# Roywangj/AdaptPoint

Hardware: AMD Instinct MI355X
Metric: set-abstraction fwd+bwd point-clouds/sec (B=32,N=1024) (higher is better)
Workload: dtype bf16

## Files before the change

adaptpoint_amd/_lib.py:

```python
import ctypes
import os

_HERE = os.path.dirname(os.path.abspath(__file__))
LIB_PATH = os.path.join(_HERE, "libadaptpoint_amd.so")
if os.environ.get("APN_LIB_PATH"):
    if os.environ.get("APN_ALLOW_UNSAFE_LIB") != "1":
        raise RuntimeError("APN_LIB_PATH is for diagnostic builds: set APN_ALLOW_UNSAFE_LIB=1 with it")
    LIB_PATH = os.path.abspath(os.environ["APN_LIB_PATH"])
REQUIRED_BUILD_FLAGS = ("-ffp-contract=off", "-fno-slp-vectorize")

_c_int, _c_float, _c_void_p = ctypes.c_int, ctypes.c_float, ctypes.c_void_p
_c_double = ctypes.c_double
_c_longlong = ctypes.c_longlong

SIGNATURES = {
    "apn_version": [],
    "apn_furthest_point_sampling": [_c_int] * 3 + [_c_void_p] * 4,
    "apn_ball_query": [_c_int] * 3 + [_c_float, _c_int] + [_c_void_p] * 4,
    "apn_group_points": [_c_int] * 5 + [_c_void_p] * 4,
    "apn_group_points_grad": [_c_int] * 5 + [_c_void_p] * 4,
    "apn_gather_points": [_c_int] * 4 + [_c_void_p] * 4,
    "apn_gather_points_grad": [_c_int] * 4 + [_c_void_p] * 4,
    "apn_resample_points": [_c_int] * 6 + [_c_void_p] * 6,
    "apn_three_nn": [_c_int] * 3 + [_c_void_p] * 5,
# ... 30 lines not shown
                       + [_c_void_p] * 3 + [_c_int] + [_c_void_p] * 8,
    "apn_sa_bwd_main": [_c_int] * 4 + [_c_float] + [_c_void_p] * 11 + [_c_double, _c_int] + [_c_void_p] * 9,
    "apn_sa_bwd_weight_rows": [_c_int] * 2,
    "apn_sa_bwd_point_grads": [_c_int] * 3 + [_c_void_p] * 7 + [_c_double, _c_int] + [_c_void_p] * 2 + [_c_int]
                              + [_c_void_p] * 4 + [_c_float] + [_c_void_p] * 5,
    "apn_sa_bwd_finalize": [_c_void_p, _c_int, _c_float, _c_void_p, _c_void_p, _c_int, _c_void_p, _c_void_p, _c_int]
                           + [_c_void_p] * 11,
    "apn_sa_forward_seq": ([_c_int] * 5 + [_c_float] + [_c_void_p] * 12
                           + [_c_void_p] * 5 + [_c_float, _c_float, _c_int]
                           + [_c_void_p] * 5 + [_c_float, _c_float, _c_int]
                           + [_c_double, _c_int] + [_c_void_p] * 11 + [_c_longlong, _c_void_p]),
    "apn_sa_backward_seq": ([_c_int] * 5 + [_c_float] + [_c_void_p] * 15 + [_c_int] * 3
                            + [_c_double] + [_c_void_p] + [_c_longlong] * 3 + [_c_void_p]
                            + [_c_longlong]
                            + [_c_void_p] * 26),
    "apn_attention_small_max": [],
    "apn_attention_small_fwd": [_c_int] * 3 + [_c_void_p] * 5,
    "apn_attention_small_bwd": [_c_int] * 3 + [_c_void_p] * 8,
    "apn_attention_prep": [_c_int] * 3 + [_c_void_p] * 4 + [_c_int, _c_void_p],
    "apn_attention_fwd": [_c_int] * 3 + [_c_void_p] * 4,
    "apn_attention_bwd": [_c_int] * 3 + [_c_void_p] * 9,
    "apn_pointset_group_rows": [_c_int] * 3,
    "apn_pointset_group_max": [_c_int] * 5 + [_c_void_p] * 8,
    "apn_pointset_group_max_grad": [_c_int] * 5 + [_c_void_p] * 9,
    "apn_sa_wide_grid": [_c_int] * 2,
    "apn_sa_wide_colsum_chunks": [_c_int] * 2,
    "apn_sa_wide_colsum": [_c_void_p, _c_int, _c_int, _c_void_p, _c_void_p, _c_void_p],
    "apn_sa_wide_tilemap_ints": [_c_int] * 2,
    "apn_sa_wide_tilemap": [_c_int] * 3 + [_c_void_p] * 3,
    "apn_sa_wide_tilemap_many": [_c_int] * 4 + [_c_void_p] * 3,
    "apn_sa_rowmap_many": [_c_int] * 4 + [_c_void_p] * 6,
    "apn_sa_rowmap_ints": [_c_int] * 2,
    "apn_sa_rowmap_places": [_c_int] * 3,
    "apn_sa_wide_stats1": [_c_int] * 4 + [_c_void_p] * 6,
    "apn_sa_wide_fwd_main": [_c_int] * 5 + [_c_void_p] * 11,
    "apn_sa_wide_bwd_main": [_c_int] * 5 + [_c_void_p] * 15,
    "apn_sa_wide_wgrad_fused": [_c_int],
    "apn_sa_wide_image": [_c_void_p, _c_int, _c_int, _c_void_p, _c_int, _c_int, _c_int, _c_void_p, _c_void_p],
    "apn_sa_wide_bwd_prep_rows": [_c_int] * 2,
    "apn_sa_wide_bwd_prep": [_c_int] * 3 + [_c_void_p] + [_c_longlong] * 3 + [_c_void_p] * 7,
    "apn_sa_wide_consts2": [_c_void_p, _c_int, _c_void_p, _c_int, _c_void_p, _c_double, _c_int] + [_c_void_p] * 4,
    "apn_sa_wide_consts1": [_c_void_p, _c_int, _c_void_p, _c_int, _c_void_p, _c_double, _c_int] + [_c_void_p] * 4,
    "apn_sa_wide_point_terms": [_c_int] * 4 + [_c_void_p] * 5 + [_c_int, _c_float] + [_c_void_p] * 7,
    "apn_sa_wide_wgrad_splits": [_c_int] * 3,
    "apn_sa_wide_csr": [_c_int] * 3 + [_c_void_p] * 9,
    "apn_sa_wide_fwd_prep": [_c_int] * 6 + [_c_float] + [_c_void_p] * 13,
    "apn_sa_wide_fwd_prep_rows": [_c_int] * 3,
    "apn_sa_wide_out": [_c_int] * 3 + [_c_void_p] * 2 + [_c_int] + [_c_void_p] * 3 + [_c_int] + [_c_void_p] * 2,
    "apn_sa_wide_bwd_mid": [_c_void_p, _c_int, _c_void_p, _c_int, _c_int, _c_void_p, _c_double, _c_int] + [_c_void_p] * 7,
    "apn_sa_wide_bwd_fin": [_c_void_p, _c_int, _c_void_p, _c_int, _c_int, _c_void_p, _c_double, _c_int] + [_c_void_p] * 8,
    "apn_sa_wide_point_grads_rows": [_c_int] * 2,
    "apn_sa_wide_point_grads_cols": [_c_int] * 3,
    "apn_sa_wide_point_grads": [_c_int] * 5 + [_c_float] + [_c_void_p] * 13 + [_c_int] + [_c_void_p] * 9,
    "apn_sa_wide_colsum_f32": [_c_void_p, _c_int, _c_int, _c_void_p, _c_void_p],
    "apn_sa_wide_wgrad": [_c_int] * 5 + [_c_void_p] * 7 + [_c_int] + [_c_void_p] * 2,
    "apn_pw_conv_tiles": [_c_int] * 2,
    "apn_pw_conv_forward": [_c_int] * 5 + [_c_void_p] * 5,
    "apn_pw_bn_act": [_c_int] * 3 + [_c_void_p] * 2 + [_c_int] + [_c_void_p] * 2 + [_c_float] * 2 + [_c_int] * 2
                     + [_c_void_p] * 6,
    "apn_pw_bn_act_grad_splits": [_c_int] * 2,
    "apn_pw_bn_act_grad": [_c_int] * 3 + [_c_void_p] * 3 + [_c_int] * 2 + [_c_void_p] * 5,
    "apn_pw_conv_grad_input": [_c_int] * 5 + [_c_void_p] * 4,
    "apn_pw_conv_grad_weight_splits": [_c_int] * 4,
    "apn_pw_conv_grad_weight": [_c_int] * 5 + [_c_void_p] * 5,
    "apn_deform_forward": [_c_int] * 3 + [_c_void_p] * 6 + [_c_float] + [_c_void_p] * 4,
    "apn_deform_backward": [_c_int] * 3 + [_c_void_p] * 4 + [_c_float] + [_c_void_p] * 7,
# ... 82 lines not shown
_lib = None


class ExtensionMissing(RuntimeError):
    pass


def load():
    global _lib
    if _lib is not None:
        return _lib
    if not os.path.exists(LIB_PATH):
        raise ExtensionMissing(
            f"{LIB_PATH} not found: build it with `python -m adaptpoint_amd.build` "
            "(hipcc --offload-arch=gfx950). There is no fallback path.")
    lib = ctypes.CDLL(LIB_PATH)
    for name, argtypes in SIGNATURES.items():
        fn = getattr(lib, name)
        fn.argtypes = argtypes
        fn.restype = _c_int
    lib.apn_error_string.argtypes = [_c_int]
    lib.apn_error_string.restype = ctypes.c_char_p
    lib.apn_build_flags.argtypes = []
    lib.apn_build_flags.restype = ctypes.c_char_p
    flags = lib.apn_build_flags().decode("utf-8", "replace").split()
    missing = [f for f in REQUIRED_BUILD_FLAGS if f not in flags]
    if missing and os.environ.get("APN_ALLOW_UNSAFE_LIB") != "1":
        raise ExtensionMissing(f"{LIB_PATH} was built without {missing} (its flags: {' '.join(flags)}): rebuild with "
                               "`python -m adaptpoint_amd.build --force`")
    _lib = lib
    return lib


def check(code, what):
    if code != 0:
        msg = load().apn_error_string(code).decode("utf-8", "replace")
        raise RuntimeError(f"{what} failed: {msg} (code {code})")
```

adaptpoint_amd/build.py:

```python
import argparse
import os
import shutil
import subprocess
import sys

HERE = os.path.dirname(os.path.abspath(__file__))
CSRC = os.path.join(HERE, "csrc")
OBJ = os.path.join(HERE, "csrc", "build")
LIB = os.path.join(HERE, "libadaptpoint_amd.so")
ARCH = "gfx950"
SOURCES = ["capi.hip", "fps.hip", "ball_query.hip", "group_points.hip", "interpolate.hip", "sa_fused.hip", "sa_glue.hip", "sa_seq.hip", "sa_geo.hip", "sa_wide.hip", "sa_wide_glue.hip", "sa_wide_dense.hip", "pointwise.hip", "feature_prop.hip", "spectral.hip", "augment.hip", "pointset_group.hip", "attention.hip", "online_aug.hip", "cloud_transform.hip", "cls_metrics.hip", "local_aggr.hip", "knn.hip", "edge_conv.hip", "chamfer.hip", "emd.hip", "pointops.hip", "point_transformer.hip", "voxel_grid.hip"]
HEADERS = ["apn_common.h", "apn_mfma.h", "sa_chain.h", "ball_query_body.h", "anchor_rotation.h", "lds_bitonic.h", "knn_list.h",
           os.path.join("..", "..", "include", "adaptpoint_amd.h")]
CXXFLAGS = ["-O3", "-std=c++17", "-fPIC", "-ffp-contract=off", "-fno-fast-math", "-fno-slp-vectorize",
            "-fvisibility=hidden", "-Wall", "-Wno-unused-command-line-argument"] + os.environ.get("APN_EXTRA_CXXFLAGS", "").split()
REQUIRED_FLAGS = ("-ffp-contract=off", "-fno-slp-vectorize")
FORBIDDEN_FLAGS = ("-fslp-vectorize", "-ffp-contract=fast", "-ffp-contract=on", "-ffast-math", "-Ofast")


NO_SLP = ["-fno-slp-vectorize"]
FILE_FLAGS = {}


def hipcc():
    exe = shutil.which("hipcc") or "/opt/rocm/bin/hipcc"
    if not os.path.exists(exe):
        raise RuntimeError("hipcc not found; libadaptpoint_amd.so cannot be built")
    return exe


def _newer(target, deps):
    if not os.path.exists(target):
        return False
    t = os.path.getmtime(target)
    return all(os.path.getmtime(d) <= t for d in deps)


def flag_line(src):
    return " ".join([*CXXFLAGS, *FILE_FLAGS.get(os.path.basename(src), [])])


def check_flags():
    bad = [f for f in CXXFLAGS if f in FORBIDDEN_FLAGS] + [f for f in REQUIRED_FLAGS if f not in CXXFLAGS]
    if bad:
# ... 56 lines not shown
```

adaptpoint_amd/csrc/capi.hip:

```cpp
#include "apn_common.h"

extern "C" int apn_version(void) { return 100;  }

#ifndef APN_BUILD_FLAGS
#define APN_BUILD_FLAGS "unknown"
#endif
extern "C" const char *apn_build_flags(void) { return APN_BUILD_FLAGS; }

extern "C" const char *apn_error_string(int code) {
    if (code == APN_OK) return "success";
    if (code == APN_EINVAL) return "invalid argument (negative size, null pointer or size beyond the launch limits)";
    return hipGetErrorString((hipError_t)code);
}

namespace apn {
__global__ void stamp_kernel(unsigned long long *stamps, int slot) { stamps[slot] = wall_clock64(); }
}

extern "C" int apn_debug_stamp(void *stamps, int slot, void *stream) {
    if (stamps == nullptr || slot < 0) return APN_EINVAL;
    hipLaunchKernelGGL(apn::stamp_kernel, dim3(1), dim3(1), 0, (hipStream_t)stream, (unsigned long long *)stamps, slot);
    return (int)hipGetLastError();
}

namespace apn {
__global__ __launch_bounds__(256) void vgpr_hold_kernel(int turns, unsigned long long *bad) {
    __shared__ unsigned long long slot[4];
    const unsigned lane = threadIdx.x;
    unsigned r[24];
#pragma unroll
    for (int i = 0; i < 24; ++i) r[i] = 0x10000u * (unsigned)(i + 1) + lane * 131u + blockIdx.x;
    if (lane < 4) slot[lane] = 0ull;
    __syncthreads();
    for (int t = 0; t < turns; ++t) {
#pragma unroll
        for (int i = 0; i < 24; ++i) asm volatile("" : "+v"(r[i]));
        if ((lane & 63) == (unsigned)(t & 63))
            atomicMax(&slot[t & 3], ((unsigned long long)r[0] << 32) | (unsigned)t);
        asm volatile("s_waitcnt lgkmcnt(0)\n\ts_barrier" ::: "memory");
        const unsigned k = (unsigned)slot[t & 3];
        if (k == 0xFFFFFFFFu) r[23] ^= 1u;
    }
#pragma unroll
    for (int i = 0; i < 24; ++i) {
// ... 91 lines not shown
```

adaptpoint_amd/fused.py:

```python
import torch
import torch.distributed as dist
import torch.nn as nn

from . import _lib
from . import ops as _ops

C_IN, C_MID, C_OUT, K_NS = 32, 32, 64, 32
DETERMINISTIC = True

PRECISION = "bf16x3"
_PREC = {"bf16": 1, "bf16x3": 2}

PER_KERNEL_LAUNCH = False


def covers(B, N, M, K, C, w1, w2, biased=False, momenta=()):
    return (C == C_IN and K == K_NS and tuple(w1) == (C_MID, C_IN + 3) and tuple(w2) == (C_OUT, C_MID) and not biased
            and (M is None or M <= N) and B <= 65535 and all(m is not None for m in momenta))


def supported(p, f, idx_or_k, conv1, conv2, bns=(), npoint=None):
    k = idx_or_k.shape[2] if torch.is_tensor(idx_or_k) else int(idx_or_k)
    m = idx_or_k.shape[1] if torch.is_tensor(idx_or_k) else npoint
    return (f.is_cuda and f.dtype == torch.float32 and p.dtype == torch.float32
            and covers(p.shape[0], p.shape[1], m, k, f.shape[1], conv1.weight.shape[:2], conv2.weight.shape[:2],
                       conv1.bias is not None or conv2.bias is not None, [bn.momentum for bn in bns]))


_FN = {}


def _call(name, dev, *args, stream=None):
    fn = _FN.get(name)
    if fn is None:
        fn = _FN[name] = getattr(_lib.load(), name)
    if stream is None:
        if dev.index is not None and dev.index != torch.cuda.current_device():
            with torch.cuda.device(dev):
                code = fn(*args, torch.cuda.current_stream(dev).cuda_stream)
            if code:
                _lib.check(code, name)
            return
        stream = torch.cuda.current_stream(dev).cuda_stream
    code = fn(*args, stream)
    if code:
        _lib.check(code, name)


class _Launcher:

    def __init__(self, dev):
        self.dev = dev
        if dev.index is not None and dev.index != torch.cuda.current_device():
            self.stream = None
        else:
            self.stream = torch.cuda.current_stream(dev).cuda_stream

    def __call__(self, name, *args):
        _call(name, self.dev, *args, stream=self.stream)


def _ptr(t):
    return None if t is None else t.data_ptr()


FORCE_PHASED = False


def _world(sync):
    if sync and dist.is_available() and dist.is_initialized():
        return dist.get_world_size()
    return 1


def _allreduce_sum_(t):
    if dist.is_available() and dist.is_initialized() and (dist.get_world_size() > 1 or FORCE_PHASED):
        from . import dp
        dp.all_reduce_sum_(t)

# ... 260 lines not shown
        need_p, need_q, a1, a2, a3, a4 = ctx.flags
        ctx.saved_tensors
        g = _backward(ctx.fw, g_out, need_p, need_q)
        ctx.fw = None
        return (g["p"], g["new_p"], g["f"], None, g["w1"], g["g1"] if a1 else None,
                g["b1"] if a2 else None, g["w2"], g["g2"] if a3 else None,
                g["b2"] if a4 else None, None)


def grouped_mlp_max(p, new_p, f, idx, radius, conv1, bn1, conv2, bn2, sync_bn=False):
    return _GroupedMlpMax.apply(p, new_p, f, idx, conv1.weight, bn1.weight, bn1.bias,
                                conv2.weight, bn2.weight, bn2.bias,
                                (radius, conv1, bn1, conv2, bn2, sync_bn))


class Sampling:

    def __init__(self, B, M, K, device):
        self.shape = (B, M, K)
        self.buf = torch.empty(B * M * (1 + 3 + K), dtype=torch.int32, device=device)
        o = 0
        self.fidx = self.buf[o:o + B * M].view(B, M)
        o += B * M
        self.new_p = self.buf[o:o + B * M * 3].view(torch.float32).view(B, M, 3)
        o += B * M * 3
        self.idx = self.buf[o:o + B * M * K].view(B, M, K)
        self.index = None
        self.tmap = None
        self.rowmap = None
        self.geo = None
        self.dd = None
        self.ready = None
        self.ties = None

    def alloc_geo(self, n_points):
        if self.geo is None or self.geo.shape[1] != n_points:
            B = self.shape[0]
            dev = self.buf.device
            self.geo = torch.empty(B, n_points, 4, dtype=torch.int64, device=dev)
            self.dd = torch.empty(B, _lib.load().apn_sa_geo_dd_doubles(n_points), dtype=torch.float64, device=dev)
        return self.geo, self.dd

    def clouds(self, lo, hi):
        v = object.__new__(Sampling)
        for name, t in vars(self).items():
            setattr(v, name, t[lo:hi] if name in _PER_CLOUD and t is not None else None)
        v.shape = (hi - lo,) + self.shape[1:]
        return v


_PER_CLOUD = ("fidx", "new_p", "idx", "geo", "dd", "ties")


@torch.no_grad()
def point_geo(p, new_p, idx, radius, out=None):
    B, N, _ = p.shape
    M, K = idx.shape[1], idx.shape[2]
    dev = p.device
    if out is None:
        geo = torch.empty(B, N, 4, dtype=torch.int64, device=dev)
        dd = torch.empty(B, _lib.load().apn_sa_geo_dd_doubles(N), dtype=torch.float64, device=dev)
    else:
        geo, dd = out
    _Launcher(dev)("apn_sa_point_geo", B, N, M, K, float(radius), p.contiguous().data_ptr(),
                   new_p.contiguous().data_ptr(), idx.contiguous().data_ptr(), geo.data_ptr(), dd.data_ptr())
    return geo, dd


@torch.no_grad()
def sample_and_query(p, npoint, radius, nsample=K_NS, out=None, geo=False, nested=False, ties=None):
    p = p.contiguous()
    dev = p.device
    B, N, _ = p.shape
    smp = out if out is not None else Sampling(B, npoint, nsample, dev)
    assert smp.shape == (B, npoint, nsample)
    gptr = dptr = None
    if geo and nsample == K_NS and smp.buf is not None:
        g_, d_ = smp.alloc_geo(N)
        gptr, dptr = g_.data_ptr(), d_.data_ptr()
    elif geo and nsample == K_NS and smp.geo is not None:
        gptr, dptr = smp.geo.data_ptr(), smp.dd.data_ptr()
    call = _Launcher(dev)
    if nested and N <= 4096:
        if smp.ties is None:
            smp.ties = torch.empty(B, dtype=torch.int32, device=dev)
        if PER_KERNEL_LAUNCH:
            call("apn_furthest_point_sampling_nested", B, N, npoint, p.data_ptr(), _ptr(ties), smp.fidx.data_ptr(),
                 smp.new_p.data_ptr(), smp.ties.data_ptr())
            call("apn_ball_query_zero", B, N, npoint, float(radius), nsample, smp.new_p.data_ptr(), p.data_ptr(),
                 smp.idx.data_ptr())
            if gptr is not None:
                call("apn_sa_point_geo", B, N, npoint, nsample, float(radius), p.data_ptr(), smp.new_p.data_ptr(),
                     smp.idx.data_ptr(), gptr, dptr)
            return smp
        call("apn_sa_sample_seq_nested", B, N, npoint, float(radius), nsample, p.data_ptr(), _ptr(ties), smp.ties.data_ptr(),
             smp.fidx.data_ptr(), smp.new_p.data_ptr(), smp.idx.data_ptr(), gptr, dptr)
        return smp
    if PER_KERNEL_LAUNCH:
        call("apn_furthest_point_sampling_xyz", B, N, npoint, p.data_ptr(), None,
             smp.fidx.data_ptr(), smp.new_p.data_ptr())
        call("apn_ball_query_zero", B, N, npoint, float(radius), nsample, smp.new_p.data_ptr(),
             p.data_ptr(), smp.idx.data_ptr())
        if gptr is not None:
            call("apn_sa_point_geo", B, N, npoint, nsample, float(radius), p.data_ptr(),
                 smp.new_p.data_ptr(), smp.idx.data_ptr(), gptr, dptr)
        return smp
    call("apn_sa_sample_seq", B, N, npoint, float(radius), nsample, p.data_ptr(), None,
         smp.fidx.data_ptr(), smp.new_p.data_ptr(), smp.idx.data_ptr(), gptr, dptr)
    return smp


@torch.no_grad()
def sample_and_query_many(ps, npoint, radius, nsample=K_NS, outs=None):
    ps = [p.contiguous() for p in ps]
    B, N, _ = ps[0].shape
    dev = ps[0].device
    if outs is None:
        outs = [Sampling(B, npoint, nsample, dev) for _ in ps]
    assert len(outs) == len(ps) and all(o.shape == (B, npoint, nsample) for o in outs)
    call = _Launcher(dev)
    for i in range(len(ps) + 1):
        a = i if i < len(ps) else None
        b = i - 1 if i >= 1 else None
        call("apn_sa_sample_overlap", B, N, npoint, float(radius), nsample,
             ps[a].data_ptr() if a is not None else None,
             outs[a].fidx.data_ptr() if a is not None else None,
             outs[a].new_p.data_ptr() if a is not None else None,
             ps[b].data_ptr() if b is not None else None,
             outs[b].new_p.data_ptr() if b is not None else None,
             outs[b].idx.data_ptr() if b is not None else None)
        if b is not None and outs[b].geo is not None:
            point_geo(ps[b], outs[b].new_p, outs[b].idx, radius, out=(outs[b].geo, outs[b].dd))
    return outs


class _SetAbstraction(torch.autograd.Function):
    @staticmethod
    def forward(ctx, p, f, w1, g1, b1, w2, g2, b2, ws, bs, mods):
        npoint, radius, conv1, bn1, conv2, bn2, skip_conv, relu, sync_bn, sampling = mods
        p = p.contiguous()
        f = f.contiguous()
        smp = sampling if sampling is not None else sample_and_query(p, npoint, radius, geo=True)
        fidx, new_p, idx = smp.fidx, smp.new_p, smp.idx
        if p.requires_grad:
            new_p = new_p.clone()
        fw = _Forward(p, f, new_p, idx, fidx, radius, conv1, bn1, conv2, bn2, skip_conv, relu,
                      sync_bn, tmap=smp.tmap, geo=smp.geo, dd=smp.dd, want_backward=any(ctx.needs_input_grad),
                      rowmap=smp.rowmap)
        ctx.fw = fw
        ctx.save_for_backward(p, f)
        ctx.set_materialize_grads(False)
        ctx.flags = (p.requires_grad, g1 is not None, b1 is not None, g2 is not None,
                     b2 is not None, ws is not None, bs is not None)
        ctx.mark_non_differentiable(new_p) if not p.requires_grad else None
        return new_p, fw.out

    @staticmethod
    def backward(ctx, g_newp_in, g_out):
        need_p, a1, a2, a3, a4, a5, a6 = ctx.flags
        fw = ctx.fw
        ctx.saved_tensors
        g = _backward(fw, g_out, need_p, need_p)
        g_p = g["p"]
        if need_p:
            gq = g["new_p"] if g_newp_in is None else g["new_p"] + g_newp_in
            g_p = g_p.scatter_add(1, fw.saved["fidx"].long().unsqueeze(-1).expand(-1, -1, 3), gq)
        ctx.fw = None
        return (g_p, g["f"], g["w1"], g["g1"] if a1 else None, g["b1"] if a2 else None, g["w2"],
                g["g2"] if a3 else None, g["b2"] if a4 else None, g["ws"] if a5 else None,
                g["bs"] if a6 else None, None)


def fused_set_abstraction(p, f, npoint, radius, conv1, bn1, conv2, bn2, skip_conv=None, relu=True,
                          sync_bn=False, sampling=None):
    assert skip_conv is None or isinstance(skip_conv, nn.Conv1d)
# ... 7 lines not shown
```

adaptpoint_amd/set_abstraction.py:

```python
import logging
from typing import NamedTuple

import torch
import torch.nn as nn

from . import fused, fused_wide, layers, pointwise
from .layers import BallGrouper, make_grouper

_log = logging.getLogger("adaptpoint_amd")

FUSED_FALLBACKS = {}


PREFER_WIDE = False
MAX_SAMPLE_SEQ_POINTS = 16384

STEM = "stem"
GROUP_ALL = "group_all"
RESIDENT = "resident"
WIDE = "wide"
GROUPED = "grouped"
COMPOSED = "composed"


# ... 142 lines not shown

    def plan(self):
        if self.is_head:
            return Plan("stem", self.fused, None, False, False, None, self.stride, None, ())
        blocks = [tuple(b) for b in self.convs]
        widths, K = tuple(b[0].out_channels for b in blocks), getattr(self.grouper, 'nsample', None)
        if self.all_aggr:
            return Plan("group_all", self.fused, None, False, False, None, self.stride, K, widths)
        skip = tuple(self.skipconv) if self.use_res and isinstance(self.skipconv, nn.Sequential) else ()
        skip = skip[0] if len(skip) == 1 and isinstance(skip[0], nn.Conv1d) and isinstance(self.act, nn.ReLU) else None
        mlp, relu_after, w1, w2, biased = None, False, None, None, False
        blk1, blk2 = blocks if len(blocks) == 2 else ((), ())
        if (isinstance(self.grouper, BallGrouper) and self.grouper.normalize_dp
                and len(blk1) == 3 and isinstance(blk1[1], nn.BatchNorm2d) and isinstance(blk1[2], nn.ReLU)
                and len(blk2) in (2, 3) and isinstance(blk2[1], nn.BatchNorm2d)
                and (len(blk2) == 2 or isinstance(blk2[2], nn.ReLU))):
            mlp, relu_after = (blk1[0], blk1[1], blk2[0], blk2[1]), len(blk2) == 3
            w1, w2 = tuple(blk1[0].weight.shape[:2]), tuple(blk2[0].weight.shape[:2])
            biased = blk1[0].bias is not None or blk2[0].bias is not None
        return Plan("ball", self.fused, mlp, relu_after, self.use_res, skip, self.stride, K, widths, w1, w2, biased)

    def route(self, c_in, B, N, cuda_f32=True, sampling=False):
        plan = self.plan()
        if c_in is None and plan.w1 is not None:
            c_in = plan.w1[1] - 3
        momenta = (plan.mlp[1].momentum, plan.mlp[3].momentum) if plan.mlp is not None else ()
        return plan, route(plan, c_in, B, N, cuda_f32, momenta, PREFER_WIDE, sampling)

    def sample(self, p, out=None, nested=False, ties=None):
        _, r = self.route(None, p.shape[0], p.shape[1], p.is_cuda and p.dtype == torch.float32, True)
        return fused.sample_and_query(p, p.shape[1] // self.stride, self.grouper.radius, self.grouper.nsample, out=out,
                                      geo=r.path == RESIDENT, nested=nested, ties=ties)

    def index_for(self, smp, n_points, c_in, out=None):
        B, M = smp.idx.shape[0], smp.idx.shape[1]
        _, r = self.route(c_in, B, n_points, smp.idx.is_cuda, True)
        if r.path == RESIDENT:
            smp.tmap = fused_wide.tile_map(smp.idx, out=smp.tmap)
            smp.rowmap = fused_wide.row_map(smp.tmap, B, n_points, M, out=smp.rowmap, fidx=smp.fidx)
        elif r.path == WIDE:
            smp.index = fused_wide.neighbour_index(smp.idx, smp.new_p, n_points, fidx=smp.fidx if r.fuse_skip else None,
                                                   out=out)
            return smp.index
        return None

    def sample_many(self, ps, outs=None):
        return fused.sample_and_query_many(ps, ps[0].shape[1] // self.stride, self.grouper.radius,
                                           self.grouper.nsample, outs=outs)

    @staticmethod
    def pool(x):
        return torch.max(x, dim=-1, keepdim=False)[0]

    def forward(self, pf, sampling=None):
        p, f = pf
        plan, r = self.route(f.shape[1], p.shape[0], p.shape[1],
                             f.is_cuda and f.dtype == torch.float32 and p.dtype == torch.float32, sampling is not None)
        if r.path == STEM:
            for blk in self.convs:
                f = pointwise.run_block(f, blk, self.fused)
            return p, f
        g, M = self.grouper, p.shape[1] // self.stride
        if r.path == RESIDENT:
            return fused.fused_set_abstraction(p, f, M, g.radius, *plan.mlp, plan.skip, plan.res or plan.relu_after,
                                               sync_bn=self.sync_bn, sampling=sampling)
        if r.path == WIDE:
            return self._wide(p, f, plan, r, sampling)
        if r.path == COMPOSED and r.reason is not None and self.sync_bn and _ranks() > 1:
            raise RuntimeError("SetAbstraction(fused=True, sync_bn=True) cannot run its fused kernels (" + r.reason +
                               ") and its BatchNorm modules are plain ones: convert them "
# ... 56 lines not shown
```

include/adaptpoint_amd.h:

```cpp
#ifndef ADAPTPOINT_AMD_H
#define ADAPTPOINT_AMD_H

#include <stddef.h>

#ifdef __cplusplus
extern "C" {
#endif

#define APN_OK 0
#define APN_EINVAL (-1)

#if defined(__GNUC__)
#define APN_API __attribute__((visibility("default")))
#else
#define APN_API
#endif

APN_API int apn_version(void);

APN_API const char *apn_error_string(int code);

APN_API const char *apn_build_flags(void);

APN_API int apn_furthest_point_sampling(int b, int n, int m, const float *xyz, float *temp,
                                int *idxs, void *stream);

APN_API int apn_ball_query(int b, int n, int m, float radius, int nsample, const float *new_xyz,
                   const float *xyz, int *idx, void *stream);

APN_API int apn_group_points(int b, int c, int n, int npoints, int nsample, const float *points,
                     const int *idx, float *out, void *stream);

APN_API int apn_group_points_grad(int b, int c, int n, int npoints, int nsample,
                          const float *grad_out, const int *idx, float *grad_points,
                          void *stream);

APN_API int apn_gather_points(int b, int c, int n, int npoints, const float *points,
                      const int *idx, float *out, void *stream);

APN_API int apn_gather_points_grad(int b, int c, int n, int npoints, const float *grad_out,
                           const int *idx, float *grad_points, void *stream);

APN_API int apn_resample_points(int b, int n, int c, int p_all, int s_cnt, int cx,
// ... 125 lines not shown
                              float *temp, int *fidx, float *new_xyz, int *idx, void *geo, void *dd,
                              void *stream);

APN_API int apn_pointset_group_rows(int b, int m, int c);
APN_API int apn_pointset_group_max(int b, int n, int m, int c, int k, const float *points,
                                   const int *idx, const int *fidx, const float *alpha,
                                   const float *beta, float *out, void *ksel, void *stream);
APN_API int apn_pointset_group_max_grad(int b, int n, int m, int c, int k, const float *points,
                                        const int *idx, const int *fidx, const float *alpha,
                                        const void *ksel, const float *g_out, float *g_points,
                                        float *part, void *stream);

APN_API int apn_attention_small_max(void);
APN_API int apn_attention_small_fwd(int b, int m, int heads, const float *q, const float *k, const float *v,
                                    float *out, void *stream);
APN_API int apn_attention_small_bwd(int b, int m, int heads, const float *q, const float *k, const float *v,
                                    const float *g_out, float *dq, float *dk, float *dv, void *stream);
APN_API int apn_attention_prep(int b, int m, int heads, const float *q, const float *k,
                               const float *v, void *images, int for_backward, void *stream);
APN_API int apn_attention_fwd(int b, int m, int heads, const void *images, float *out, float *lse,
                              void *stream);
APN_API int apn_attention_bwd(int b, int m, int heads, const void *images, const float *out,
                              const float *lse, const float *g_out, void *scratch, float *dq,
                              float *dk, float *dv, void *stream);

APN_API int apn_sa_wide_grid(int b, int m);
APN_API int apn_sa_wide_tilemap_ints(int b, int m);
APN_API int apn_sa_wide_tilemap(int b, int m, int mode, const int *idx, int *tmap, void *stream);
APN_API int apn_sa_wide_tilemap_many(int count, int b, int m, int mode, const int *idx, int *tmap, void *stream);
APN_API int apn_sa_rowmap_places(int b, int n, int m);
APN_API int apn_sa_rowmap_ints(int b, int n);
APN_API int apn_sa_rowmap_many(int count, int b, int n, int m, const int *tmap, const int *fidx, int *pcnt_poff, int *rowdst, int *scratch,
                               void *stream);
APN_API int apn_sa_wide_colsum_chunks(int rows, int ncol);
APN_API int apn_sa_wide_colsum(const float *part, int rows, int ncol, double *scratch, double *out,
                               void *stream);
APN_API int apn_sa_wide_stats1(int b, int n, int m, int c_mid, const float *U, const float *V,
                               const int *idx, const int *tmap, float *part, void *stream);
APN_API int apn_sa_wide_fwd_main(int b, int n, int m, int c_mid, int c_out, const float *U, const float *V,
                                 const int *idx, const int *tmap, const void *w2_image, const float *pack1,
                                 const float *sgn2, float *ysel, void *ksel, float *part, void *stream);
APN_API int apn_sa_wide_bwd_main(int b, int n, int m, int c_mid, int c_out, const float *U, const float *V,
                                 const int *idx, const int *tmap, const void *z_image, const float *pack1,
                                 const float *evec, const float *goa, const void *ksel, float *GU,
                                 float *HA, float *HB, float *part, float *r_part, void *stream);
APN_API int apn_sa_wide_wgrad_fused(int c_mid);
APN_API int apn_sa_wide_image(const float *src0, int k0, int trans0, const float *src1, int kd, int nc, int ct,
                              void *image, void *stream);
APN_API int apn_sa_wide_bwd_prep_rows(int b, int m);
APN_API int apn_sa_wide_bwd_prep(int b, int m, int c_out, const float *g, long long gs_b, long long gs_c,
                                 long long gs_m, const float *ysel, const float *pack2, const float *out_act,
                                 float *gpre, float *goa, float *part_s, void *stream);
APN_API int apn_sa_wide_consts2(const float *part_s, int rows, const double *sums, int c_out,
                                const float *pack2, double count, int training, float *d2e2,
                                float *g_gamma2, float *g_beta2, void *stream);
APN_API int apn_sa_wide_consts1(const float *part_t, int rows, const double *sums, int c_mid,
                                const float *pack1, double count, int training, float *cabc,
                                float *g_gamma1, float *g_beta1, void *stream);
APN_API int apn_sa_wide_point_terms(int b, int n, int m, int c_mid, const float *cabc, const float *pack1,
                                    const float *U, const float *geo, const float *w1, int ldw, float radius,
                                    const float *GU, const int *pcnt_poff, const int *plist, float *G, float *HA,
                                    const float *HB, void *stream);
APN_API int apn_sa_wide_wgrad_splits(int b, int m, int c_mid);
APN_API int apn_sa_wide_wgrad(int b, int n, int m, int c_mid, int c_out, const float *U, const float *V,
                              const int *idx, const int *tmap, const float *pack1, const float *goa,
                              const void *ksel, int splits, float *r_part, void *stream);
// ... 244 lines not shown
```

Baseline: 121,300.

## Fuse point-geometry stats, tile map and row map into two per-cloud kernels

Adds an index-tail entry that computes per-point geometry sums, covariance stats, tile map and row map in two one-workgroup-per-cloud kernels held in LDS, replacing the separate point_geo, tile_map and row_map launches on the training path. The goal is fewer launches and less global-memory round-tripping of intermediate index data. The fallback to the old entries stays for shapes that do not fit, signalled by a new not-applicable code. It adds a lot of complex scan and binary-lifting logic, and the large per-block LDS and one-block-per-cloud grid may limit parallelism.

```diff
diff --git a/adaptpoint_amd/_lib.py b/adaptpoint_amd/_lib.py
--- a/adaptpoint_amd/_lib.py
+++ b/adaptpoint_amd/_lib.py
@@ -86,6 +86,8 @@
     "apn_sa_rowmap_many": [_c_int] * 4 + [_c_void_p] * 6,
     "apn_sa_rowmap_ints": [_c_int] * 2,
     "apn_sa_rowmap_places": [_c_int] * 3,
+    "apn_sa_index_tail": [_c_int] * 4 + [_c_float] + [_c_void_p] * 10,
+    "apn_sa_index_tail_many": [_c_int] * 5 + [_c_float] + [_c_void_p] * 10,
     "apn_sa_wide_stats1": [_c_int] * 4 + [_c_void_p] * 6,
     "apn_sa_wide_fwd_main": [_c_int] * 5 + [_c_void_p] * 11,
     "apn_sa_wide_bwd_main": [_c_int] * 5 + [_c_void_p] * 15,
@@ -234,6 +236,9 @@
     return lib
 
 
+NOT_APPLICABLE = -2
+
+
 def check(code, what):
     if code != 0:
         msg = load().apn_error_string(code).decode("utf-8", "replace")
diff --git a/adaptpoint_amd/build.py b/adaptpoint_amd/build.py
--- a/adaptpoint_amd/build.py
+++ b/adaptpoint_amd/build.py
@@ -9,7 +9,7 @@
 OBJ = os.path.join(HERE, "csrc", "build")
 LIB = os.path.join(HERE, "libadaptpoint_amd.so")
 ARCH = "gfx950"
-SOURCES = ["capi.hip", "fps.hip", "ball_query.hip", "group_points.hip", "interpolate.hip", "sa_fused.hip", "sa_glue.hip", "sa_seq.hip", "sa_geo.hip", "sa_wide.hip", "sa_wide_glue.hip", "sa_wide_dense.hip", "pointwise.hip", "feature_prop.hip", "spectral.hip", "augment.hip", "pointset_group.hip", "attention.hip", "online_aug.hip", "cloud_transform.hip", "cls_metrics.hip", "local_aggr.hip", "knn.hip", "edge_conv.hip", "chamfer.hip", "emd.hip", "pointops.hip", "point_transformer.hip", "voxel_grid.hip"]
+SOURCES = ["capi.hip", "fps.hip", "ball_query.hip", "group_points.hip", "interpolate.hip", "sa_fused.hip", "sa_glue.hip", "sa_seq.hip", "sa_geo.hip", "sa_index_tail.hip", "sa_wide.hip", "sa_wide_glue.hip", "sa_wide_dense.hip", "pointwise.hip", "feature_prop.hip", "spectral.hip", "augment.hip", "pointset_group.hip", "attention.hip", "online_aug.hip", "cloud_transform.hip", "cls_metrics.hip", "local_aggr.hip", "knn.hip", "edge_conv.hip", "chamfer.hip", "emd.hip", "pointops.hip", "point_transformer.hip", "voxel_grid.hip"]
 HEADERS = ["apn_common.h", "apn_mfma.h", "sa_chain.h", "ball_query_body.h", "anchor_rotation.h", "lds_bitonic.h", "knn_list.h",
            os.path.join("..", "..", "include", "adaptpoint_amd.h")]
 CXXFLAGS = ["-O3", "-std=c++17", "-fPIC", "-ffp-contract=off", "-fno-fast-math", "-fno-slp-vectorize",
diff --git a/adaptpoint_amd/csrc/capi.hip b/adaptpoint_amd/csrc/capi.hip
--- a/adaptpoint_amd/csrc/capi.hip
+++ b/adaptpoint_amd/csrc/capi.hip
@@ -10,6 +10,7 @@
 extern "C" const char *apn_error_string(int code) {
     if (code == APN_OK) return "success";
     if (code == APN_EINVAL) return "invalid argument (negative size, null pointer or size beyond the launch limits)";
+    if (code == APN_ENOTAPPLICABLE) return "the entry's one-workgroup kernels do not fit this shape (use the entries it stands for)";
     return hipGetErrorString((hipError_t)code);
 }
 
diff --git a/adaptpoint_amd/csrc/sa_index_tail.hip b/adaptpoint_amd/csrc/sa_index_tail.hip
--- /dev/null
+++ b/adaptpoint_amd/csrc/sa_index_tail.hip
@@ -0,0 +1,498 @@
+#include "apn_common.h"
+
+namespace apn {
+
+constexpr double TAIL_GEO_UNIT = 68719476736.0;
+constexpr int TAIL_INS = 16;
+
+__device__ __forceinline__ int scan1024(int v, int *wtot, int &total) {
+    const int lane = threadIdx.x & 63, wave = threadIdx.x >> 6;
+    int incl = v;
+#pragma unroll
+    for (int d = 1; d < 64; d <<= 1) {
+        const int o = __shfl_up(incl, d);
+        if (lane >= d) incl += o;
+    }
+    __syncthreads();
+    if (lane == 63) wtot[wave] = incl;
+    __syncthreads();
+    int before = 0;
+    total = 0;
+#pragma unroll
+    for (int w = 0; w < 16; ++w) {
+        const int x = wtot[w];
+        before += w < wave ? x : 0;
+        total += x;
+    }
+    return incl + before;
+}
+
+__global__ __launch_bounds__(1024) void index_stats_pack_kernel(
+    int n, int m, int levels, int u_bytes, float radius, const float *__restrict__ xyz,
+    const float *__restrict__ new_xyz, const int *__restrict__ idx, long long *__restrict__ geo,
+    double *__restrict__ dd, int *__restrict__ pcnt, unsigned char *__restrict__ cnt8, unsigned *__restrict__ qmeta,
+    int *__restrict__ tcount, unsigned short *__restrict__ tnq_local, long long blob_bytes, long long rowmap_ints) {
+    extern __shared__ unsigned long long tail_lds[];
+    __shared__ float red[16][6];
+    __shared__ int wtot[16];
+    __shared__ int ntile_s;
+    {
+        const long long z = blockIdx.y, b = gridDim.x, off = z * blob_bytes;
+        xyz += z * b * n * 3;
+        new_xyz += z * b * m * 3;
+        idx += z * b * m * 32;
+        geo += z * b * n * 4;
+        dd += z * b * 6;
+        pcnt += z * rowmap_ints;
+        cnt8 += off;
+        qmeta = reinterpret_cast<unsigned *>(reinterpret_cast<char *>(qmeta) + off);
+        tcount = reinterpret_cast<int *>(reinterpret_cast<char *>(tcount) + off);
+        tnq_local = reinterpret_cast<unsigned short *>(reinterpret_cast<char *>(tnq_local) + off);
+    }
+    unsigned long long *acc = tail_lds;
+    int *scn = reinterpret_cast<int *>(reinterpret_cast<char *>(tail_lds) + u_bytes);
+    int *spc = scn + m;
+    float *sp = reinterpret_cast<float *>(spc + n);
+    float *sq = sp + 3 * n;
+    const int tid = threadIdx.x, lane = tid & 63, wave = tid >> 6, k = lane & 31, half = lane >> 5;
+    const int cloud = blockIdx.x;
+    constexpr int PF = 16;
+    int nbv[PF];
+    auto request = [&](int qb0) {
+#pragma unroll
+        for (int u = 0; u < PF; ++u) {
+            const int q = qb0 + 32 * u + half;
+            nbv[u] = idx[((size_t)cloud * m + (q < m ? q : 0)) * 32 + k];
+        }
+    };
+    request(wave * 2);
+    for (int e = tid; e < n * 3; e += 1024) sp[e] = xyz[(size_t)cloud * n * 3 + e];
+    for (int e = tid; e < m * 3; e += 1024) sq[e] = new_xyz[(size_t)cloud * m * 3 + e];
+    for (int e = tid; e < n * 4; e += 1024) acc[e] = 0ull;
+    for (int e = tid; e < n; e += 1024) spc[e] = 0;
+    __syncthreads();
+    float v[6] = {0.f, 0.f, 0.f, 0.f, 0.f, 0.f};
+    for (int qb0 = wave * 2; qb0 < m; qb0 += 32 * PF) {
+        if (qb0 != wave * 2) request(qb0);
+#pragma unroll
+        for (int u = 0; u < PF; ++u) {
+            const int qb = qb0 + 32 * u;
+            if (qb >= m) break;
+            const int q = qb + half;
+            const bool live_q = q < m;
+            const int nb = nbv[u];
+            const int nb0 = __shfl(nb, half * 32);
+            const bool fill = k > 0 && nb == nb0;
+            const unsigned long long bal = __ballot(fill);
+            const int nfill = __popc((unsigned)(bal >> (32 * half)));
+            const int mult = !live_q ? 0 : (k == 0 ? 1 + nfill : (fill ? 0 : 1));
+            const unsigned differ = (unsigned)(__ballot(nb != nb0) >> (32 * half));
+            const int c = __popc(differ) + 1;
+            const int cn = differ == ((c >= 32 ? 0xffffffffu : ((1u << c) - 1u)) & ~1u) ? c : 32;
+            if (live_q && k == 0) scn[q] = cn;
+            if (live_q && k < cn && (unsigned)nb < (unsigned)n) atomicAdd(&spc[nb], 1);
+            if (mult && nb >= 0 && nb < n) {
+                const float *p = sp + (size_t)nb * 3;
+                const float *qq = sq + (size_t)q * 3;
+                const float dx = (p[0] - qq[0]) / radius, dy = (p[1] - qq[1]) / radius, dz = (p[2] - qq[2]) / radius;
+                unsigned long long *g = acc + (size_t)nb * 4;
+                const long long mm = mult;
+                atomicAdd(g, (unsigned long long)mm);
+                atomicAdd(g + 1, (unsigned long long)(mm * __double2ll_rn((double)dx * TAIL_GEO_UNIT)));
+                atomicAdd(g + 2, (unsigned long long)(mm * __double2ll_rn((double)dy * TAIL_GEO_UNIT)));
+                atomicAdd(g + 3, (unsigned long long)(mm * __double2ll_rn((double)dz * TAIL_GEO_UNIT)));
+                const float fm = (float)mult;
+                v[0] += fm * dx * dx; v[1] += fm * dx * dy; v[2] += fm * dx * dz;
+                v[3] += fm * dy * dy; v[4] += fm * dy * dz; v[5] += fm * dz * dz;
+            }
+        }
+    }
+#pragma unroll
+    for (int j = 0; j < 6; ++j) {
+#pragma unroll
+        for (int s = 1; s < 64; s <<= 1) v[j] += __shfl_xor(v[j], s);
+        if (lane == 0) red[wave][j] = v[j];
+    }
+    __syncthreads();
+    {
+        ulonglong2 *dst = reinterpret_cast<ulonglong2 *>(geo + (size_t)cloud * n * 4);
+        const ulonglong2 *src = reinterpret_cast<const ulonglong2 *>(acc);
+        for (int e = tid; e < n * 2; e += 1024) dst[e] = src[e];
+        for (int e = tid; e < n; e += 1024) pcnt[(size_t)cloud * n + e] = spc[e];
+    }
+    if (tid < 6) {
+        double s = 0.0;
+#pragma unroll
+        for (int w = 0; w < 16; ++w) s += (double)red[w][tid];
+        dd[(size_t)cloud * 6 + tid] = s;
+    }
+    __syncthreads();
+
+    int *P = reinterpret_cast<int *>(tail_lds);
+    int *start = P + (m + 1);
+    int *jump = start + (m + 1);
+    const int t = tid;
+    const int per = (m + 1023) / 1024;
+    int cnq[2], loc = 0;
+#pragma unroll
+    for (int i = 0; i < 2; ++i) {
+        const int q = t * per + i;
+        cnq[i] = (i < per && q < m) ? scn[q] : 0;
+        loc += cnq[i];
+    }
+    int total;
+    int run = scan1024(loc, wtot, total) - loc;
+#pragma unroll
+    for (int i = 0; i < 2; ++i) {
+        const int q = t * per + i;
+        if (i < per && q < m) {
+            P[q] = run;
+            cnt8[(size_t)cloud * m + q] = (unsigned char)cnq[i];
+            run += cnq[i];
+        }
+    }
+    if (t == 0) { P[m] = total; ntile_s = 0; }
+    __syncthreads();
+    for (int q = t; q <= m; q += 1024) {
+        int nx = m;
+        if (q < m) {
+            const int lim = P[q] + 32;
+            int lo = q + 1, hi = m;
+            while (lo < hi) {
+                const int mid = (lo + hi) >> 1;
+                if (P[mid + 1] > lim) hi = mid; else lo = mid + 1;
+            }
+            nx = lo;
+        }
+        jump[q] = nx;
+    }
+    __syncthreads();
+    for (int kk = 1; kk < levels; ++kk) {
+        int *prev = jump + (kk - 1) * (m + 1), *cur = jump + kk * (m + 1);
+        for (int q = t; q <= m; q += 1024) cur[q] = prev[prev[q]];
+        __syncthreads();
+    }
+    for (int tl = t; tl <= m; tl += 1024) {
+        int s0 = 0;
+        for (int kk = 0; kk < levels; ++kk)
+            if ((tl >> kk) & 1) s0 = jump[kk * (m + 1) + s0];
+        start[tl] = tl < m ? s0 : m;
+    }
+    __syncthreads();
+    for (int tl = t; tl < m; tl += 1024) {
+        if (start[tl] < m) {
+            const int nxt = start[tl + 1];
+            tnq_local[(size_t)cloud * m + tl] = (unsigned short)(nxt - start[tl]);
+            if (nxt >= m) ntile_s = tl + 1;
+        }
+    }
+    __syncthreads();
+    const int T = ntile_s;
+    if (t == 0) tcount[cloud] = T;
+    for (int q = t; q < m; q += 1024) {
+        int lo = 0, hi = T - 1;
+        while (lo < hi) {
+            const int mid = (lo + hi + 1) >> 1;
+            if (start[mid] <= q) lo = mid; else hi = mid - 1;
+        }
+        const int s0 = start[lo];
+        qmeta[(size_t)cloud * m + q] = (unsigned)lo | ((unsigned)(P[q] - P[s0]) << 16) | (q == s0 ? 1u << 24 : 0u) |
+                                       ((unsigned)(q - s0) << 25);
+    }
+}
+
+__global__ __launch_bounds__(1024) void index_rows_map_kernel(
+    int b, int n, int m, const int *__restrict__ idx, const int *__restrict__ fidx,
+    const unsigned char *__restrict__ cnt8, const unsigned *__restrict__ qmeta, const int *__restrict__ tcount,
+    int *__restrict__ toff, const unsigned short *__restrict__ tnq_local, int *__restrict__ ntiles,
+    int *__restrict__ tq0, unsigned *__restrict__ rowinfo, int *__restrict__ rownn, int *__restrict__ pcnt_poff,
+    int *__restrict__ rowdst, int rows_cap, int bitonic_words, long long blob_bytes, long long rowmap_ints) {
+    extern __shared__ int rows_lds[];
+    __shared__ int wtot[16];
+    __shared__ unsigned marks[1024];
+    __shared__ int nlong, sdup;
+    {
+        const long long z = blockIdx.y, off = z * blob_bytes;
+        idx += z * b * m * 32;
+        if (fidx) fidx += z * b * m;
+        cnt8 += off;
+        qmeta = reinterpret_cast<const unsigned *>(reinterpret_cast<const char *>(qmeta) + off);
+        tcount = reinterpret_cast<const int *>(reinterpret_cast<const char *>(tcount) + off);
+        toff = reinterpret_cast<int *>(reinterpret_cast<char *>(toff) + off);
+        tnq_local = reinterpret_cast<const unsigned short *>(reinterpret_cast<const char *>(tnq_local) + off);
+        ntiles = reinterpret_cast<int *>(reinterpret_cast<char *>(ntiles) + off);
+        tq0 = reinterpret_cast<int *>(reinterpret_cast<char *>(tq0) + off);
+        rowinfo = reinterpret_cast<unsigned *>(reinterpret_cast<char *>(rowinfo) + off);
+        rownn = reinterpret_cast<int *>(reinterpret_cast<char *>(rownn) + off);
+        pcnt_poff += z * rowmap_ints;
+        rowdst += z * 32 * b * m;
+    }
+    int *scur = rows_lds, *soff = scur + n, *slist = soff + n;
+    int *slong = slist + rows_cap;
+    int *scn = slong + rows_cap / TAIL_INS + 1;
+    unsigned *smeta = reinterpret_cast<unsigned *>(scn + m);
+    int *stnq = reinterpret_cast<int *>(smeta + m);
+    int *sbit = stnq + m;
+    const int c = blockIdx.x, t = threadIdx.x, lane = t & 63, wave = t >> 6, l32 = lane & 31, half = lane >> 5;
+    const size_t cbase = (size_t)c * n;
+    const int *pcnt = pcnt_poff;
+    int *poff = pcnt_poff + (size_t)b * n, *dup = pcnt_poff + 2 * (size_t)b * n;
+
+    constexpr int QW = 16;
+    int nbv[QW];
+    auto request = [&](int qb0) {
+#pragma unroll
+        for (int j = 0; j < QW; ++j) {
+            const int ql = qb0 + wave * 2 * QW + 2 * j + half;
+            nbv[j] = idx[((size_t)c * m + (ql < m ? ql : m - 1)) * 32 + l32];
+        }
+    };
+    request(0);
+    int tsum = 0;
+    for (int j = t; j < c; j += 1024) tsum += tcount[j];
+    const int tmine = tcount[c];
+    const int per = (n + 1023) / 1024;
+    int pc[2];
+#pragma unroll
+    for (int i = 0; i < 2; ++i) {
+        const int k = t * per + i;
+        pc[i] = (i < per && k < n) ? pcnt[cbase + k] : 0;
+    }
+    const bool marking = fidx != nullptr && n <= 32 * 1024;
+    const int pick = (marking && t < m) ? fidx[(size_t)c * m + t] : 0;
+    if (t < m) {
+        scn[t] = cnt8[(size_t)c * m + t];
+        smeta[t] = qmeta[(size_t)c * m + t];
+        stnq[t] = tnq_local[(size_t)c * m + t];
+    }
+    marks[t] = 0u;
+    if (t == 0) { nlong = 0; sdup = 0; }
+
+    int base_tile;
+    (void)scan1024(tsum, wtot, base_tile);
+    const int row0 = base_tile * 32;
+    if (t == 0) {
+        toff[c] = base_tile;
+        if (c == b - 1) ntiles[0] = base_tile + tmine;
+    }
+    const int sum = pc[0] + pc[1];
+    int total;
+    int run = scan1024(sum, wtot, total) - sum;
+#pragma unroll
+    for (int i = 0; i < 2; ++i) {
+        const int k = t * per + i;
+        if (i < per && k < n) {
+            soff[k] = run;
+            scur[k] = run;
+            poff[cbase + k] = row0 + run;
+            if (pc[i] > TAIL_INS) slong[atomicAdd(&nlong, 1)] = k;
+            run += pc[i];
+        }
+    }
+    if (marking && t < m) {
+        const unsigned bit = 1u << (pick & 31);
+        if ((atomicOr(&marks[(pick >> 5) & 1023], bit) & bit) != 0u) sdup = 1;
+    }
+    if (t < m) {
+        const unsigned meta = smeta[t];
+        const bool ends = t == m - 1 || ((smeta[t + 1 < m ? t + 1 : t] >> 24) & 1);
+        scn[t] = scn[t] | (ends ? 1 << 8 : 0) | (stnq[meta & 0xffff] << 16);
+    }
+    __syncthreads();
+    if (t == 0) dup[c] = marking ? sdup : 1;
+
+    for (int qb0 = 0; qb0 < m; qb0 += 32 * QW) {
+        if (qb0 != 0) request(qb0);
+        unsigned wa[QW], wb[QW];
+#pragma unroll
+        for (int j = 0; j < QW; ++j) {
+            const int ql = qb0 + wave * 2 * QW + 2 * j + half;
+            wa[j] = smeta[ql < m ? ql : m - 1];
+            wb[j] = (unsigned)scn[ql < m ? ql : m - 1];
+        }
+#pragma unroll
+        for (int j = 0; j < QW; ++j) {
+            const int ql = qb0 + wave * 2 * QW + 2 * j + half;
+            const int nb = nbv[j];
+            const int nb0 = __shfl(nb, half * 32);
+            if (ql >= m) continue;
+            const size_t q = (size_t)c * m + ql;
+            const unsigned meta = wa[j];
+            const int cn = wb[j] & 0xff;
+            const bool ends = (wb[j] >> 8) & 1;
+            const int tl = meta & 0xffff, r0 = (meta >> 16) & 0xff;
+            const bool starts = (meta >> 24) & 1;
+            const size_t tile = (size_t)base_tile + tl;
+            const unsigned qlocal = (meta >> 25) & 0x3fu;
+            if (l32 < cn) {
+                const unsigned mult = l32 == 0 ? (unsigned)(33 - cn) : 1u;
+                unsigned v = qlocal | ((unsigned)l32 << 8) | (mult << 16);
+                if (starts && l32 == 0) v |= (wb[j] >> 16) << 24;
+                rowinfo[tile * 32 + r0 + l32] = v;
+                rownn[tile * 32 + r0 + l32] = nb;
+                if ((unsigned)nb < (unsigned)n) {
+                    const unsigned e = (unsigned)(tl * 32 + r0 + l32);
+                    slist[atomicAdd(&scur[nb], 1)] = (int)((e << 16) | (mult << 10) | (unsigned)ql);
+                }
+            }
+            if (ends && r0 + cn + l32 < 32) {
+                rowinfo[tile * 32 + r0 + cn + l32] = 0xffu;
+                rownn[tile * 32 + r0 + cn + l32] = nb0;
+            }
+            if (starts && l32 == 0) tq0[tile] = (int)q;
+        }
+    }
+    __syncthreads();
+    for (int k = t; k < n; k += 1024) {
+        const int st = soff[k], cnt = scur[k] - st;
+        if (cnt > TAIL_INS || cnt < 2) continue;
+        int *l = slist + st;
+        int r[TAIL_INS];
+#pragma unroll
+        for (int i = 0; i < TAIL_INS; ++i) r[i] = i < cnt ? l[i] : 0x7fffffff;
+#pragma unroll
+        for (int kk = 2; kk <= TAIL_INS; kk <<= 1) {
+#pragma unroll
+            for (int j = kk >> 1; j > 0; j >>= 1) {
+#pragma unroll
+                for (int i = 0; i < TAIL_INS; ++i) {
+                    const int o = i ^ j;
+                    if (o > i) {
+                        const int x = r[i], y = r[o];
+                        const int lo = x < y ? x : y, hi = x < y ? y : x;
+                        r[i] = (i & kk) == 0 ? lo : hi;
+                        r[o] = (i & kk) == 0 ? hi : lo;
+                    }
+                }
+            }
+        }
+#pragma unroll
+        for (int i = 0; i < TAIL_INS; ++i)
+            if (i < cnt) l[i] = r[i];
+    }
+    for (int li = wave; li < nlong; li += 16) {
+        const int k = slong[li], st = soff[k], cnt = scur[k] - st;
+        int *l = slist + st;
+        if (cnt <= 64) {
+            int v = lane < cnt ? l[lane] : 0x7fffffff;
+#pragma unroll
+            for (int kk = 2; kk <= 64; kk <<= 1) {
+#pragma unroll
+                for (int j = kk >> 1; j > 0; j >>= 1) {
+                    const int o = __shfl_xor(v, j);
+                    const bool up = (lane & kk) == 0, low = (lane & j) == 0;
+                    v = (low == up) ? (v < o ? v : o) : (v > o ? v : o);
+                }
+            }
+            if (lane < cnt) l[lane] = v;
+            continue;
+        }
+        if (cnt <= bitonic_words) {
+            int nn2 = 128;
+            while (nn2 < cnt) nn2 <<= 1;
+            int *bb = sbit + wave * bitonic_words;
+            for (int i = lane; i < nn2; i += 64) bb[i] = i < cnt ? l[i] : 0x7fffffff;
+            for (int kk = 2; kk <= nn2; kk <<= 1) {
+                for (int j = kk >> 1; j > 0; j >>= 1) {
+                    for (int t2 = lane; t2 < nn2 / 2; t2 += 64) {
+                        const int i = ((t2 & ~(j - 1)) << 1) | (t2 & (j - 1));
+                        const int pp = i | j;
+                        const bool up = (i & kk) == 0;
+                        const int x = bb[i], y = bb[pp];
+                        if ((x > y) == up) { bb[i] = y; bb[pp] = x; }
+                    }
+                }
+            }
+            for (int i = lane; i < cnt; i += 64) l[i] = bb[i];
+            continue;
+        }
+        int mine[16], rank[16];
+        const int cc = cnt < 1024 ? cnt : 1024;
+#pragma unroll
+        for (int u = 0; u < 16; ++u) {
+            const int i = lane + 64 * u;
+            mine[u] = i < cc ? l[i] : 0x7fffffff;
+            rank[u] = 0;
+        }
+        for (int j = 0; j < cc; ++j) {
+            const int v = l[j];
+#pragma unroll
+            for (int u = 0; u < 16; ++u)
+                if (64 * u < cc) rank[u] += v < mine[u] ? 1 : 0;
+        }
+        asm volatile("s_waitcnt lgkmcnt(0)" ::: "memory");
+#pragma unroll
+        for (int u = 0; u < 16; ++u)
+            if (lane + 64 * u < cc) l[rank[u]] = mine[u];
+    }
+    __syncthreads();
+    for (int i = t; i < total; i += 1024) rowdst[row0 + (int)((unsigned)slist[i] >> 16)] = row0 + i;
+}
+
+struct TailPlan {
+    int levels, u_bytes, bitonic_words;
+    size_t lds_a, lds_b;
+    bool ok;
+};
+
+static TailPlan tail_plan(int n, int m) {
+    TailPlan p = {};
+    if (apn_sa_geo_dd_doubles(n) != 6 || n > 2048 || m > 2048) return p;
+    p.levels = 1;
+    while ((1 << p.levels) <= m) ++p.levels;
+    const size_t acc = (size_t)n * 32, pack = (size_t)(p.levels + 2) * (m + 1) * 4;
+    p.u_bytes = (int)(((acc > pack ? acc : pack) + 15) & ~(size_t)15);
+    p.lds_a = (size_t)p.u_bytes + 16 * ((size_t)m + n);
+    const long long rows_cap = (long long)m * 32;
+    const long long csr = 4 * (2ll * n + rows_cap + 3ll * m + rows_cap / TAIL_INS + 1);
+    if (m > 1024 || rows_cap > 65536 || csr > 150 * 1024 || p.lds_a > 150 * 1024) return p;
+    const long long mine = 4 * (2ll * n + rows_cap + rows_cap / TAIL_INS + 1 + 3ll * m);
+    for (int wds = 1024; wds >= 128; wds >>= 1)
+        if (mine + 16ll * wds * 4 <= 150 * 1024) { p.bitonic_words = wds; break; }
+    p.lds_b = (size_t)(mine + 16ll * p.bitonic_words * 4);
+    p.ok = true;
+    return p;
+}
+
+}
+
+extern "C" int apn_sa_index_tail_many(int count, int b, int n, int m, int nsample, float radius, const float *xyz,
+                                      const float *new_xyz, const int *idx, const int *fidx, void *geo, void *dd,
+                                      int *tmap, int *pcnt_poff, int *rowdst, void *stream) {
+    using namespace apn;
+    if (count <= 0 || count > 65535 || b <= 0 || n <= 0 || m <= 0 || nsample != 32 || b > 65535 || !(radius > 0.0f) ||
+        (long long)b * m > 0x7fffffffLL / 64 || (long long)b * n > 0x7fffffffLL / 8 || 32ll * b * m > 0x7fffffffLL / 128)
+        return APN_EINVAL;
+    if (!xyz || !new_xyz || !idx || !geo || !dd || !tmap || !pcnt_poff || !rowdst || ((uintptr_t)geo & 15))
+        return APN_EINVAL;
+    const TailPlan plan = tail_plan(n, m);
+    if (!plan.ok) return APN_ENOTAPPLICABLE;
+    const int nq = b * m;
+    const long long blob_bytes = (long long)apn_sa_wide_tilemap_ints(b, m) * 4, rowmap_ints = apn_sa_rowmap_ints(b, n);
+    int *tq0 = tmap + 4;
+    unsigned *rowinfo = (unsigned *)(tmap + 4 + (size_t)((nq + 3) & ~3));
+    int *rownn = (int *)(rowinfo + (size_t)32 * nq);
+    int *tcount = rownn + (size_t)32 * nq, *toff = tcount + b;
+    unsigned *qmeta = (unsigned *)(toff + b);
+    unsigned short *tnq_local = (unsigned short *)(qmeta + nq);
+    unsigned char *cnt8 = (unsigned char *)(tnq_local + 2 * (((size_t)nq + 1) / 2));
+    hipStream_t st = (hipStream_t)stream;
+    static DynLdsOnce conf_a, conf_b;
+    if (hipError_t e = set_dyn_lds(conf_a, (const void *)index_stats_pack_kernel, 150 * 1024)) return (int)e;
+    if (hipError_t e = set_dyn_lds(conf_b, (const void *)index_rows_map_kernel, 150 * 1024)) return (int)e;
+    hipLaunchKernelGGL(index_stats_pack_kernel, dim3(b, count), dim3(1024), plan.lds_a, st, n, m, plan.levels,
+                       plan.u_bytes, radius, xyz, new_xyz, idx, (long long *)geo, (double *)dd, pcnt_poff, cnt8, qmeta,
+                       tcount, tnq_local, blob_bytes, rowmap_ints);
+    hipLaunchKernelGGL(index_rows_map_kernel, dim3(b, count), dim3(1024), plan.lds_b, st, b, n, m, idx, fidx, cnt8,
+                       qmeta, tcount, toff, tnq_local, tmap, tq0, rowinfo, rownn, pcnt_poff, rowdst, m * 32,
+                       plan.bitonic_words, blob_bytes, rowmap_ints);
+    APN_LAUNCH_CHECK();
+    return APN_OK;
+}
+
+extern "C" int apn_sa_index_tail(int b, int n, int m, int nsample, float radius, const float *xyz, const float *new_xyz,
+                                 const int *idx, const int *fidx, void *geo, void *dd, int *tmap, int *pcnt_poff,
+                                 int *rowdst, void *stream) {
+    return apn_sa_index_tail_many(1, b, n, m, nsample, radius, xyz, new_xyz, idx, fidx, geo, dd, tmap, pcnt_poff, rowdst,
+                                  stream);
+}
diff --git a/adaptpoint_amd/fused.py b/adaptpoint_amd/fused.py
--- a/adaptpoint_amd/fused.py
+++ b/adaptpoint_amd/fused.py
@@ -30,7 +30,7 @@
 _FN = {}
 
 
-def _call(name, dev, *args, stream=None):
+def _call(name, dev, *args, stream=None, allow=()):
     fn = _FN.get(name)
     if fn is None:
         fn = _FN[name] = getattr(_lib.load(), name)
@@ -38,13 +38,14 @@
         if dev.index is not None and dev.index != torch.cuda.current_device():
             with torch.cuda.device(dev):
                 code = fn(*args, torch.cuda.current_stream(dev).cuda_stream)
-            if code:
+            if code and code not in allow:
                 _lib.check(code, name)
-            return
+            return code
         stream = torch.cuda.current_stream(dev).cuda_stream
     code = fn(*args, stream)
-    if code:
+    if code and code not in allow:
         _lib.check(code, name)
+    return code
 
 
 class _Launcher:
@@ -371,6 +372,7 @@
         self.dd = None
         self.ready = None
         self.ties = None
+        self.stats_pending = False
 
     def alloc_geo(self, n_points):
         if self.geo is None or self.geo.shape[1] != n_points:
@@ -407,12 +409,43 @@
 
 
 @torch.no_grad()
+def index_tail(p, smp, radius):
+    from . import fused_wide
+    p = p.contiguous()
+    dev = p.device
+    B, N, _ = p.shape
+    M, K = smp.idx.shape[1], smp.idx.shape[2]
+    lib = _lib.load()
+    if smp.geo is None or smp.geo.shape[1] != N:
+        smp.geo = torch.empty(B, N, 4, dtype=torch.int64, device=dev)
+        smp.dd = torch.empty(B, lib.apn_sa_geo_dd_doubles(N), dtype=torch.float64, device=dev)
+    if smp.tmap is None:
+        smp.tmap = torch.empty(lib.apn_sa_wide_tilemap_ints(B, M), dtype=torch.int32, device=dev)
+    if smp.rowmap is None:
+        smp.rowmap = (torch.empty(lib.apn_sa_rowmap_ints(B, N), dtype=torch.int32, device=dev),
+                      torch.empty(32 * B * M, dtype=torch.int32, device=dev))
+    code = _lib.NOT_APPLICABLE
+    if K == K_NS:
+        args = (B, N, M, K, float(radius), p.data_ptr(), smp.new_p.data_ptr(), smp.idx.data_ptr(), smp.fidx.data_ptr(),
+                smp.geo.data_ptr(), smp.dd.data_ptr(), smp.tmap.data_ptr(), smp.rowmap[0].data_ptr(),
+                smp.rowmap[1].data_ptr())
+        code = _call("apn_sa_index_tail", dev, *args, allow=(_lib.NOT_APPLICABLE,))
+    if code != 0:
+        point_geo(p, smp.new_p, smp.idx, radius, out=(smp.geo, smp.dd))
+        fused_wide.tile_map(smp.idx, out=smp.tmap)
+        fused_wide.row_map(smp.tmap, B, N, M, out=smp.rowmap, fidx=smp.fidx)
+    smp.stats_pending = False
+    return code == 0
+
+
+@torch.no_grad()
 def sample_and_query(p, npoint, radius, nsample=K_NS, out=None, geo=False, nested=False, ties=None):
     p = p.contiguous()
     dev = p.device
     B, N, _ = p.shape
     smp = out if out is not None else Sampling(B, npoint, nsample, dev)
     assert smp.shape == (B, npoint, nsample)
+    smp.stats_pending = not geo
     gptr = dptr = None
     if geo and nsample == K_NS and smp.buf is not None:
         g_, d_ = smp.alloc_geo(N)
@@ -479,7 +512,13 @@
         npoint, radius, conv1, bn1, conv2, bn2, skip_conv, relu, sync_bn, sampling = mods
         p = p.contiguous()
         f = f.contiguous()
-        smp = sampling if sampling is not None else sample_and_query(p, npoint, radius, geo=True)
+        if sampling is not None:
+            smp = sampling
+        elif any(ctx.needs_input_grad):
+            smp = sample_and_query(p, npoint, radius, geo=False)
+            index_tail(p, smp, radius)
+        else:
+            smp = sample_and_query(p, npoint, radius, geo=True)
         fidx, new_p, idx = smp.fidx, smp.new_p, smp.idx
         if p.requires_grad:
             new_p = new_p.clone()
diff --git a/adaptpoint_amd/set_abstraction.py b/adaptpoint_amd/set_abstraction.py
--- a/adaptpoint_amd/set_abstraction.py
+++ b/adaptpoint_amd/set_abstraction.py
@@ -198,10 +198,12 @@
         return fused.sample_and_query(p, p.shape[1] // self.stride, self.grouper.radius, self.grouper.nsample, out=out,
                                       geo=r.path == RESIDENT, nested=nested, ties=ties)
 
-    def index_for(self, smp, n_points, c_in, out=None):
+    def index_for(self, smp, n_points, c_in, out=None, p=None):
         B, M = smp.idx.shape[0], smp.idx.shape[1]
         _, r = self.route(c_in, B, n_points, smp.idx.is_cuda, True)
-        if r.path == RESIDENT:
+        if r.path == RESIDENT and smp.stats_pending and p is not None:
+            fused.index_tail(p, smp, self.grouper.radius)
+        elif r.path == RESIDENT:
             smp.tmap = fused_wide.tile_map(smp.idx, out=smp.tmap)
             smp.rowmap = fused_wide.row_map(smp.tmap, B, n_points, M, out=smp.rowmap, fidx=smp.fidx)
         elif r.path == WIDE:
diff --git a/include/adaptpoint_amd.h b/include/adaptpoint_amd.h
--- a/include/adaptpoint_amd.h
+++ b/include/adaptpoint_amd.h
@@ -9,6 +9,7 @@
 
 #define APN_OK 0
 #define APN_EINVAL (-1)
+#define APN_ENOTAPPLICABLE (-2)
 
 #if defined(__GNUC__)
 #define APN_API __attribute__((visibility("default")))
@@ -200,6 +201,12 @@
 APN_API int apn_sa_rowmap_ints(int b, int n);
 APN_API int apn_sa_rowmap_many(int count, int b, int n, int m, const int *tmap, const int *fidx, int *pcnt_poff, int *rowdst, int *scratch,
                                void *stream);
+APN_API int apn_sa_index_tail(int b, int n, int m, int nsample, float radius, const float *xyz, const float *new_xyz,
+                              const int *idx, const int *fidx, void *geo, void *dd, int *tmap, int *pcnt_poff, int *rowdst,
+                              void *stream);
+APN_API int apn_sa_index_tail_many(int count, int b, int n, int m, int nsample, float radius, const float *xyz,
+                                   const float *new_xyz, const int *idx, const int *fidx, void *geo, void *dd, int *tmap,
+                                   int *pcnt_poff, int *rowdst, void *stream);
 APN_API int apn_sa_wide_colsum_chunks(int rows, int ncol);
 APN_API int apn_sa_wide_colsum(const float *part, int rows, int ncol, double *scratch, double *out,
                                void *stream);
```

Result: no change. 121,600 (median of 4 runs) (+0.2%).
